# roymor1/OptimalStrategiesAgainstGenerativeAttacks

Measured on AMD Instinct MI355X. Metric: GIM episodes/sec (64x64x3, m=1 n=5 k=10), higher is better.
Workload: dtype f32

## Files before the change

### optimalstrategiesagainstgenerativeattacks_amd/csrc/conv_igemm.hip

```cpp
#include <stdlib.h>

#include "common.h"
#include <type_traits>

#define PM_MAX_PIXELS 16
#define PM_MIN_IMAGES 32
#define BK 16

struct Geo {
    int N, H, W, logH, logW;
    int Hin, Win;
    int ups;
    int s_in;
    int s_in_x;
    int off_y, off_x;
    int Th, Tw;
    int KF;
    int KFw;
    int wa_base, wa_step, wb_base, wb_step;
    int os, py, px;
    int pc, pc_kind, pc_K;
    int pm;
    unsigned long long pm_perm;
    unsigned long long pm_perm_cls[4];
// ... 1377 lines not shown

__global__ __launch_bounds__(256) void xfold_weights_kernel(const float* __restrict__ w, float* __restrict__ wx, int Cout, int Cin, int K, int J) {
    const int KW = K + J - 1;
    const long long total = (long long)J * Cin * K * KW * Cout;
    for (long long i = (long long)blockIdx.x * 256 + threadIdx.x; i < total; i += (long long)gridDim.x * 256) {
        const int co = (int)(i % Cout);
        long long r = i / Cout;
        const int u = (int)(r % KW); r /= KW;
        const int a = (int)(r % K); r /= K;
        const int ci = (int)(r % Cin), j = (int)(r / Cin);
        const int b = u - j;
        wx[i] = (b >= 0 && b < K) ? w[(((long long)co * K + (K - 1 - a)) * K + (K - 1 - b)) * Cin + ci] : 0.f;
    }
}

extern "C" int gim_conv2d_xfold_weights(const float* w, float* wx, int Cout, int Cin, int KH, int J, void* stream) {
    GIM_CHECK_ARG(w && wx && Cout > 0 && Cin > 0 && KH > 0 && (KH & 1) && J >= 2 && (J & (J - 1)) == 0, "xfold_weights: bad args");
    const long long total = (long long)J * Cin * KH * (KH + J - 1) * Cout;
    const int blocks = (int)((total + 255) / 256 < 2048 ? (total + 255) / 256 : 2048);
    hipLaunchKernelGGL(xfold_weights_kernel, dim3(blocks), dim3(256), 0, (hipStream_t)stream, w, wx, Cout, Cin, KH, J);
    return gim_check_launch("gim_conv2d_xfold_weights");
}

static int check_shape(const gim_conv_shape* s) {
    GIM_CHECK_ARG(s != nullptr, "conv: null shape");
    GIM_CHECK_ARG(s->N > 0 && s->Cin > 0 && s->Cout > 0, "conv: non-positive dims");
    GIM_CHECK_ARG(s->KH > 0 && (s->KH & 1), "conv: KH must be odd");
    GIM_CHECK_ARG(s->ups == 0 || s->ups == 1, "conv: ups must be 0 or 1");
    GIM_CHECK_ARG(ilog2_exact(s->H) >= 0 && ilog2_exact(s->W) >= 0, "conv: H and W must be powers of two");
    GIM_CHECK_ARG(!s->ups || (s->H >= 2 && s->W >= 2), "conv: ups needs H, W >= 2");
    GIM_CHECK_ARG(!s->pool || (!s->ups && s->H >= 2 && s->W >= 2 && s->wfold), "conv: pool needs ups == 0, H, W >= 2 and folded weights");
    GIM_CHECK_ARG(!s->wfold || s->pool || s->ups, "conv: wfold only with pool or ups");
    GIM_CHECK_ARG((long long)s->N * s->H * s->W < (1ll << 31), "conv: too many output pixels");
    GIM_CHECK_ARG(s->prec >= 0 && s->prec <= 2, "conv: prec must be 0 (fp32 MFMA), 1 (fp16 operands, fp32 accumulate; saturating) or 2 (the same, non-saturating)");
    return GIM_OK;
}

static void geo_grid(Geo& g, int N, int H, int W) {
    g.N = N; g.H = H; g.W = W; g.logH = ilog2_exact(H); g.logW = ilog2_exact(W);
}

static Geo geo_plain(const gim_conv_shape* s, bool flip) {
    Geo g{};
    const int pad = (s->KH - 1) / 2;
    geo_grid(g, s->N, s->H, s->W);
    g.ups = flip ? 0 : s->ups;
    g.Hin = s->H >> g.ups; g.Win = s->W >> g.ups;
    g.s_in = g.s_in_x = 1; g.off_y = g.off_x = -pad; g.Th = g.Tw = g.KF = g.KFw = s->KH;
    g.wa_base = g.wb_base = flip ? s->KH - 1 : 0;
    g.wa_step = g.wb_step = flip ? -1 : 1;
    g.os = 1;
    return g;
// ... 299 lines not shown
static int fwd_call(ConvCall& c, const float* x, const float* w, const float* bias, const float* sigma, const float* residual, float* y,
                    const gim_conv_shape* s) {
    c = ConvCall{};
    ConvP& p = c.p;
    const bool up_fold = s->ups && s->wfold;
    int rc = convp_begin(p, s->pool ? geo_s2(s, false) : (up_fold ? geo_pc(s, 0) : geo_plain(s, false)), s->Cin, s->Cout, s->Cin, 0, s,
                         "conv: one image of the gathered tensor exceeds 2 GiB (32-bit buffer offsets)");
    if (rc) return rc;
    p.x = x; p.w = w; p.bias = bias; p.sigma = sigma; p.res = residual; p.mask_x = nullptr; p.y = y;
    p.Cin_w = s->Cin;
    p.pre_slope = s->pre_slope; p.mask_slope = 1.f; p.out_scale = s->pool ? 0.25f : 1.f; p.res_ups = s->res_ups;
    GIM_CHECK_ARG(s->post_slope >= 0.f && s->post_slope <= 1.f, "conv fwd: post_slope must be in [0, 1] (0 or 1 = none)");
    p.post_slope = (s->post_slope > 0.f) ? s->post_slope : 1.f;
    p.f16 = s->prec;
    c.y_elems = (size_t)s->N * (s->H >> s->pool) * (s->W >> s->pool) * s->Cout;
    GIM_CHECK_ARG(c.y_elems * sizeof(float) <= 0x7FFFFFF0ull, "conv: one image of the output exceeds 2 GiB (32-bit buffer offsets)");
    c.bmode = 0;
    c.gen = ((s->Cin % BK) != 0 || ((uintptr_t)x & 15) || ((uintptr_t)w & 15)) ? 1 : 0;
    return GIM_OK;
}

extern "C" int gim_conv2d_fwd(const float* x, const float* w, const float* bias, const float* sigma, const float* residual,
                              float* y, const gim_conv_shape* s, void* stream) {
    int rc = check_shape(s);
    if (rc) return rc;
    GIM_CHECK_ARG(x && w && y, "conv fwd: null pointer");
    if (tiny_route(s)) {
        gim_tiny_fwd(x, w, bias, sigma, residual, y, s, (hipStream_t)stream);
        return gim_check_launch("gim_conv2d_fwd");
    }
    size_t xi, yi;
    image_elems(s, false, xi, yi);
    gim_conv_shape a, b;
    if (split_batch(*s, xi > yi ? xi : yi, a, b)) {
        const size_t ri = s->res_ups ? yi / 4 : yi;
        rc = gim_conv2d_fwd(x, w, bias, sigma, residual, y, &a, stream);
        if (rc) return rc;
        return gim_conv2d_fwd(x + a.N * xi, w, bias, sigma, residual ? residual + a.N * ri : nullptr, y + a.N * yi, &b, stream);
    }
    ConvCall c;
    rc = fwd_call(c, x, w, bias, sigma, residual, y, s);
    return rc ? rc : plan_and_run(c, stream, "gim_conv2d_fwd");
}

static Geo geo_strided(const gim_infer_conv* s) {
    Geo g{};
    const int pad = (s->KH - 1) / 2;
// ... 49 lines not shown
    if (rc) return rc;
    p.x = dy; p.w = w; p.bias = nullptr; p.sigma = sigma; p.res = res_half; p.res_scale = res_scale; p.mask_x = mask_x; p.y = dx;
    p.Cin_w = s->Cin;
    p.pre_slope = 1.f; p.mask_slope = s->pre_slope; p.out_scale = s->pool ? 0.25f : 1.f; p.res_ups = 0;
    p.post_slope = 1.f;
    c.y_elems = (size_t)s->N * (s->H >> (up_fold ? 1 : 0)) * (s->W >> (up_fold ? 1 : 0)) * s->Cin;
    GIM_CHECK_ARG(c.y_elems * sizeof(float) <= 0x7FFFFFF0ull, "conv: one image of the output exceeds 2 GiB (32-bit buffer offsets)");
    const bool gen = (s->Cout % BK) != 0 || ((uintptr_t)dy & 15);
    const bool bscalar = (s->Cin % 4) != 0 || ((uintptr_t)w & 15);
    p.f16 = transposed ? s->prec : 0;
    if (transposed) {
        GIM_CHECK_ARG(!gen && !((uintptr_t)w & 15), "conv dgrad (transposed weights): Cout % 16 == 0 and 16-byte aligned operands required");
        p.Cin_w = s->Cout;
        p.tune_kind = 4;
        c.bmode = 0; c.gen = 0;
    } else {
        c.bmode = 1; c.gen = (gen ? 1 : 0) | (bscalar ? 2 : 0);
    }
    return GIM_OK;
}

static int dgrad_impl(const float* dy, const float* w, const float* sigma, const float* mask_x, float* dx,
                      const gim_conv_shape* s, void* stream, bool transposed, const float* res_half = nullptr, float res_scale = 0.f) {
    int rc = check_shape(s);
    if (rc) return rc;
    GIM_CHECK_ARG(dy && w && dx, "conv dgrad: null pointer");
    if (!transposed && !res_half && tiny_route(s)) {
        gim_tiny_dgrad(dy, w, sigma, mask_x, dx, s, (hipStream_t)stream);
        return gim_check_launch("gim_conv2d_dgrad");
    }
    size_t xi, yi;
    image_elems(s, true, xi, yi);
    gim_conv_shape a, b;
    if (split_batch(*s, xi > yi ? xi : yi, a, b)) {
        rc = dgrad_impl(dy, w, sigma, mask_x, dx, &a, stream, transposed, res_half, res_scale);
        if (rc) return rc;
        return dgrad_impl(dy + a.N * yi, w, sigma, mask_x ? mask_x + a.N * xi : nullptr, dx + a.N * xi, &b, stream, transposed,
                          res_half ? res_half + a.N * (xi / 4) : nullptr, res_scale);
    }
    ConvCall c;
    rc = dgrad_call(c, dy, w, sigma, mask_x, dx, s, transposed, res_half, res_scale);
    return rc ? rc : plan_and_run(c, stream, transposed ? "gim_conv2d_dgrad_t" : "gim_conv2d_dgrad");
}

extern "C" int gim_conv2d_dgrad(const float* dy, const float* w, const float* sigma, const float* mask_x, float* dx,
                                const gim_conv_shape* s, void* stream) {
    return dgrad_impl(dy, w, sigma, mask_x, dx, s, stream, false);
// ... 230 lines not shown
            for (int m = m0 + lane; m < m1; m += 64) sb += nar[(long long)m * Cn + part];
        if (part < 8) red[0][part][lane] = sb;
        __syncthreads();
        if (threadIdx.x < Cn) {
            float v = 0.f;
            for (int q = 0; q < 64; ++q) v += red[0][threadIdx.x][q];
            atomicAdd(&bias_out[threadIdx.x], v);
        }
    }
}

enum WgFamily { WG_MFMA = 0, WG_MFMA_F16, WG_TINY, WG_ROW, WG_NARROW };
enum WgCombine { WG_SLABS = 0, WG_ONE_SLAB, WG_ACC };
struct WgPlan {
    int family;
    int rows, cols, M;
    int ns;
    int atomic;
    int bm, bn, bk, xcd;
    int slices, mper;
    int gx, gy, gz;
    int table_hit;
};

static WgPlan wgrad_plan(const gim_conv_shape* s0, bool rows_form, int combine, bool aligned) {
    WgPlan q{};
    gim_conv_shape v = *s0;
    if (rows_form) {
        v.tune_tile = s0->tune_tile ? s0->tune_tile : -1;
        v.prec = 0;
    }
    const gim_conv_shape* s = &v;
    const bool up_fold = s->ups && s->wfold;
    const int KF = s->wfold ? s->KH + 1 : s->KH;
    q.rows = up_fold ? s->Cin : s->Cout;
    q.cols = KF * KF * (up_fold ? s->Cout : s->Cin);
    const long long M = (long long)s->N * (s->H >> (s->wfold ? 1 : 0)) * (s->W >> (s->wfold ? 1 : 0));
    q.M = (int)M;
    int target = s->tune_wgrad > 0 ? s->tune_wgrad : 0;
    int tile = s->tune_tile > 0 ? s->tune_tile : 0;
    if (!target && !tile && s->tune_tile == 0) {
        const int pcw = (s->pool ? 1 : 0) + (up_fold ? 2 : 0);
        const TuneEntry* te = tune_lookup(2, (int)M, q.rows, q.cols, s->KH, pcw);
        if (te) { target = te->ks; tile = te->tile; q.table_hit = 1; }
    }
    bool row_resident = false;
// ... 12 lines not shown
    const long long tiles = (long long)((q.cols + q.bn - 1) / q.bn) * ((q.rows + q.bm - 1) / q.bm);
    long long minpix = 512;
    if (!target) {
        target = 1024;
        if (tiles * ((M + 511) / 512) < 256) minpix = 128;
    } else {
        minpix = 64;
    }
    long long S = (target + tiles - 1) / tiles;
    const long long maxS = (M + minpix - 1) / minpix;
    if (S > maxS) S = maxS;
    if (S > 1024) S = 1024;
    if (S < 1) S = 1;
    long long mp = (M + S - 1) / S;
    mp = (mp + q.bk - 1) / q.bk * q.bk;
    q.ns = (int)((M + mp - 1) / mp);
    if (rows_form) {
        q.cols = s->KH * ((s->KH * s->Cin + 15) & ~15);
        q.bn = (q.bm == 32 || q.cols > 64) ? 128 : 64;
    }
    q.atomic = combine == WG_ACC || (combine == WG_ONE_SLAB && q.ns > 1);
    const bool plain = !rows_form && !s->wfold && !s->ups && !s->pool;
    const bool untuned = s->tune_tile == 0 && s->tune_wgrad == 0;
    if (!rows_form && combine != WG_SLABS && untuned && gim_tiny_shape(s)) {
        const dim3 g = gim_tiny_grid(s);
        q.family = WG_TINY;
        q.table_hit = q.bm = q.bn = 0;
        q.gx = g.x; q.gy = g.y; q.gz = 1;
        q.slices = q.gx * q.gy;
    } else if (plain && row_resident && q.atomic && s->KH == 3 && s->Cin % 32 == 0 && s->Cout % 128 == 0 && s->H * s->W >= 16 && s->W >= 4 && aligned) {
        q.family = WG_ROW;
        q.bm = 128; q.bn = 96;
        q.gx = 3 * (s->Cin / 32); q.gy = s->Cout / 128;
        const int wgs = q.gx * q.gy;
        long long Sr = ((row_target > 0 ? row_target : 1024) + wgs - 1) / wgs;
        const long long maxSr = (M + 127) / 128;
        if (Sr > maxSr) Sr = maxSr;
        if (Sr < 1) Sr = 1;
        mp = (M + Sr - 1) / Sr;
        mp = (mp + 15) / 16 * 16;
        q.slices = q.gz = (int)((M + mp - 1) / mp);
    } else if (plain && s->KH == 1 && q.atomic && (s->Cin <= 8 || s->Cout <= 8) && (s->Cin >= 16 || s->Cout >= 16) && M % NARROW_U == 0 && untuned) {
        q.family = WG_NARROW;
        q.table_hit = q.bm = q.bn = 0;
        mp = NARROW_MPER;
        q.slices = q.gx = (int)((M + NARROW_MPER - 1) / NARROW_MPER);
        q.gy = ((s->Cin <= 8 ? s->Cout : s->Cin) + 63) / 64;
        q.gz = 1;
    } else {
        q.family = f16 ? WG_MFMA_F16 : WG_MFMA;
        q.slices = q.ns;
        q.xcd = (q.ns >= 64 || (q.ns >= 8 && q.ns % 8 == 0)) ? 1 : 0;
        q.gx = (q.cols + q.bn - 1) / q.bn; q.gy = (q.rows + q.bm - 1) / q.bm;
        q.gz = q.xcd ? (q.ns + 7) / 8 * 8 : q.ns;
    }
    q.mper = (int)mp;
    return q;
}

extern "C" int gim_conv2d_wgrad_slabs(const gim_conv_shape* s) {
    if (check_shape(s)) return GIM_E_BADARG;
    return wgrad_plan(s, false, WG_SLABS, true).ns;
}

static int wgrad_call(WgP& p, WgPlan& q, const float* dy, const float* x, float* slabs, float* bias_slabs, int n_slabs, const gim_conv_shape* s,
                      bool prezeroed, bool rows) {
    int rc = check_shape(s);
    if (rc) return rc;
    GIM_CHECK_ARG(dy && x && slabs, "conv wgrad: null pointer");
    q = wgrad_plan(s, rows, prezeroed ? WG_ACC : (n_slabs == 1 ? WG_ONE_SLAB : WG_SLABS), !((uintptr_t)dy & 15) && !((uintptr_t)x & 15));
    if (!prezeroed) GIM_CHECK_ARG(n_slabs == 1 || n_slabs == q.ns, "conv wgrad: n_slabs must be 1 (atomic combine) or gim_conv2d_wgrad_slabs(shape)");
    const bool up_fold = s->ups && s->wfold;
    GIM_CHECK_ARG(!(up_fold && bias_slabs), "conv wgrad: the sub-pixel form does not produce the bias gradient (use gim_colsum)");
    p = WgP{};
    p.zero = zero_page();
    p.pos_inf = __builtin_inff();
    if (rows) p.g = geo_rows(s);
    else if (s->pool || up_fold) p.g = geo_s2(s, false);
    else p.g = geo_plain(s, false);
    if (up_fold) {
        p.dy = x; p.x = dy; p.Cin = s->Cout; p.Cout = s->Cin; p.pre_slope = 1.f; p.a_slope = s->pre_slope; p.pix = s->Cout;
    } else {
        p.dy = dy; p.x = x; p.Cin = s->Cin; p.Cout = s->Cout; p.pre_slope = s->pre_slope; p.a_slope = 1.f; p.pix = s->Cin;
    }
    p.slabs = slabs; p.bias_slabs = bias_slabs;
    p.M = q.M; p.Kcols = q.cols; p.mper = q.mper; p.ns = q.slices; p.xcd = q.xcd; p.atomic = q.atomic;
    if (rows) { p.Cin = (s->KH * s->Cin + 15) & ~15; p.pix = s->Cin; p.pre_slope = 1.f; }
    const unsigned long long xb = (unsigned long long)p.g.N * p.g.Hin * p.g.Win * p.pix * 4ull;
    GIM_CHECK_ARG(xb <= 0x7FFFFFF0ull, "conv wgrad: gathered tensor larger than 2 GiB (32-bit buffer offsets): split the batch");
    p.x_bytes = (unsigned)xb;
    return GIM_OK;
}

// ... 32 lines not shown
        const bool va = (p.Cout % 4 == 0) && !((uintptr_t)p.dy & 15);
        const bool vb = (p.Cin % 4 == 0) && !((uintptr_t)p.x & 15);
        const int bk = (q.bk == 32 && va && vb) ? 32 : BK;
        const bool fastb = vb && p.g.ups == 0 && ((p.g.H * p.g.W) & (bk - 1)) == 0;
        const bool f16 = q.family == WG_MFMA_F16 && va && vb && bk == 32, sat = s->prec != 2;
        if (f16 && fastb) hipLaunchKernelGGL((sat ? conv_wgrad_f16_kernel<true, true> : conv_wgrad_f16_kernel<true, false>), g, dim3(256), 0, st, p);
        else if (f16) hipLaunchKernelGGL((sat ? conv_wgrad_f16_kernel<false, true> : conv_wgrad_f16_kernel<false, false>), g, dim3(256), 0, st, p);
        else if (va && fastb) launch_wgrad<4, 4, true>(p, q.bm, q.bn, bk, g, st);
        else if (va && vb) launch_wgrad<4, 4, false>(p, q.bm, q.bn, bk, g, st);
        else if (va) launch_wgrad<4, 1, false>(p, q.bm, q.bn, bk, g, st);
        else if (vb) launch_wgrad<1, 4, false>(p, q.bm, q.bn, bk, g, st);
        else launch_wgrad<1, 1, false>(p, q.bm, q.bn, bk, g, st);
    }
    }
    return gim_check_launch("gim_conv2d_wgrad");
}

extern "C" int gim_conv2d_wgrad(const float* dy, const float* x, float* slabs, float* bias_slabs, int n_slabs,
                                const gim_conv_shape* s, void* stream) {
    return wgrad_impl(dy, x, slabs, bias_slabs, n_slabs, s, stream, false);
}

extern "C" int gim_conv2d_wgrad_acc(const float* dy, const float* x, float* acc, float* bias_acc, const gim_conv_shape* s, void* stream) {
    int rc = check_shape(s);
    if (rc) return rc;
    size_t xi, yi;
    image_elems(s, false, xi, yi);
    gim_conv_shape a, b;
    if (split_batch(*s, xi > yi ? xi : yi, a, b)) {
        rc = gim_conv2d_wgrad_acc(dy, x, acc, bias_acc, &a, stream);
        if (rc) return rc;
        return gim_conv2d_wgrad_acc(dy + a.N * yi, x + a.N * xi, acc, bias_acc, &b, stream);
    }
    return wgrad_impl(dy, x, acc, bias_acc, 1, s, stream, true);
}

extern "C" int gim_conv2d_wgrad_rows_acc(const float* dy, const float* xp, float* acc, float* bias_acc, const gim_conv_shape* s, void* stream) {
    int rc = rows_shape_ok(s);
    if (rc) return rc;
    GIM_CHECK_ARG(s->Cout % 4 == 0 && dy && xp && !((uintptr_t)dy & 15) && !((uintptr_t)xp & 15), "conv wgrad (rows form): Cout % 4 == 0 and 16-byte aligned operands required");
    return wgrad_impl(dy, xp, acc, bias_acc, 1, s, stream, true, true);
}

static void plan_row(int32_t* out, int table_hit, int bm, int bn, int slices, int gx, int gy, int gz, int form) {
    const int32_t v[8] = {table_hit, bm, bn, slices, gx, gy, gz, form};
    for (int i = 0; i < 8; ++i) out[i] = v[i];
}
// ... 42 lines not shown
```

### optimalstrategiesagainstgenerativeattacks_amd/csrc/conv_tiny.hip

```cpp
#include "common.h"

struct TinyP {
    const float* in;
    const float* w;
    const float* bias;
    const float* sigma;
    const float* res;
    float* out;
    float* out2;
    int N, H, W;
    float pre_slope;
    float post_slope;
    int res_ups;
};

constexpr int TT = GIM_TINY_TILE;

template <int K, int CI, int CO, bool FLIP>
__global__ __launch_bounds__(256) void conv_tiny_kernel(const TinyP p) {
    constexpr int PAD = (K - 1) / 2, TW = TT + K - 1;
    constexpr int CG = FLIP ? CO : CI, CP = FLIP ? CI : CO;
    __shared__ float xs[TW * TW * CG];
    const int t = threadIdx.x;
    const int tiles_x = (p.W + TT - 1) / TT;
    const int oy0 = (blockIdx.x / tiles_x) * TT, ox0 = (blockIdx.x % tiles_x) * TT, n = blockIdx.y;
    const float* img = p.in + (long long)n * p.H * p.W * CG;
    for (int idx = t; idx < TW * TW * CG; idx += 256) {
        const int c = idx % CG, rc = idx / CG, col = rc % TW, row = rc / TW;
        const int iy = oy0 + row - PAD, ix = ox0 + col - PAD;
        float v = 0.f;
        if ((unsigned)iy < (unsigned)p.H && (unsigned)ix < (unsigned)p.W) v = img[((long long)iy * p.W + ix) * CG + c];
        if (!FLIP) v = fmaxf(v, v * p.pre_slope);
        xs[idx] = v;
    }
    __syncthreads();
    const int ty = t >> 4, tx = t & 15;
    float acc[CP];
#pragma unroll
    for (int c = 0; c < CP; ++c) acc[c] = 0.f;
    for (int ta = 0; ta < K; ++ta) {
#pragma unroll
        for (int tb = 0; tb < K; ++tb) {
// ... 9 lines not shown
            }
        }
    }
    const int oy = oy0 + ty, ox = ox0 + tx;
    if (oy >= p.H || ox >= p.W) return;
    const float scale = p.sigma ? 1.0f / p.sigma[0] : 1.0f;
    const long long o = (((long long)n * p.H + oy) * p.W + ox) * CP;
#pragma unroll
    for (int c = 0; c < CP; ++c) {
        float v = acc[c] * scale;
        if (FLIP) {
            if (p.res) v *= (p.res[o + c] > 0.f ? 1.0f : p.pre_slope);
        } else {
            if (p.bias) v += p.bias[c];
            if (p.res) v += p.res_ups ? p.res[(((long long)n * (p.H >> 1) + (oy >> 1)) * (p.W >> 1) + (ox >> 1)) * CP + c] : p.res[o + c];
            v = fmaxf(v, v * p.post_slope);
        }
        p.out[o + c] = v;
    }
}

template <int K, int CI, int CO>
__global__ __launch_bounds__(256) void conv_tiny_wgrad_kernel(const TinyP p) {
    constexpr int PAD = (K - 1) / 2, TW = TT + K - 1, NT = K * K * CI, G = 256 / NT;
    static_assert(G >= 1, "one thread per (tap, channel)");
    __shared__ float xs[TW * TW * CI];
    __shared__ float dys[TT * TT * CO];
    const int t = threadIdx.x;
    const int tiles_x = (p.W + TT - 1) / TT;
    const int oy0 = (blockIdx.x / tiles_x) * TT, ox0 = (blockIdx.x % tiles_x) * TT, n = blockIdx.y;
    const float* img = p.in + (long long)n * p.H * p.W * CI;
    const float* dyi = p.res + (long long)n * p.H * p.W * CO;
    for (int idx = t; idx < TW * TW * CI; idx += 256) {
        const int c = idx % CI, rc = idx / CI, col = rc % TW, row = rc / TW;
        const int iy = oy0 + row - PAD, ix = ox0 + col - PAD;
        float v = 0.f;
        if ((unsigned)iy < (unsigned)p.H && (unsigned)ix < (unsigned)p.W) v = img[((long long)iy * p.W + ix) * CI + c];
        xs[idx] = fmaxf(v, v * p.pre_slope);
    }
    for (int idx = t; idx < TT * TT * CO; idx += 256) {
        const int c = idx % CO, pp = idx / CO, oy = oy0 + (pp >> 4), ox = ox0 + (pp & 15);
        dys[idx] = (oy < p.H && ox < p.W) ? dyi[((long long)oy * p.W + ox) * CO + c] : 0.f;
    }
    __syncthreads();
    __shared__ float red[256 * CO];
    if (t < G * NT) {
        const int grp = t / NT, id = t - grp * NT;
        const int ci = id % CI, tap = id / CI, tb = tap % K, ta = tap / K;
        float acc[CO];
#pragma unroll
        for (int c = 0; c < CO; ++c) acc[c] = 0.f;
        for (int pp = grp; pp < TT * TT; pp += G) {
            const float xv = xs[(((pp >> 4) + ta) * TW + (pp & 15) + tb) * CI + ci];
#pragma unroll
            for (int c = 0; c < CO; ++c) acc[c] += dys[pp * CO + c] * xv;
        }
#pragma unroll
        for (int c = 0; c < CO; ++c) red[(grp * NT + id) * CO + c] = acc[c];
    }
    __syncthreads();
    for (int o = t; o < NT * CO; o += 256) {
        const int id = o / CO, c = o - id * CO;
        float v = 0.f;
        for (int gq = 0; gq < G; ++gq) v += red[(gq * NT + id) * CO + c];
        const int ci = id % CI, tap = id / CI, tb = tap % K, ta = tap / K;
        atomicAdd(&p.out[((c * K + ta) * K + tb) * CI + ci], v);
    }
    if (p.out2 && t >= 256 - CO) {
        const int c = t - (256 - CO);
        float s = 0.f;
        for (int pp = 0; pp < TT * TT; ++pp) s += dys[pp * CO + c];
        atomicAdd(&p.out2[c], s);
    }
}

bool gim_tiny_shape(const gim_conv_shape* s) {
    if (s->N > 65535) return false;
    return !s->ups && !s->pool && !s->wfold && s->Cin == s->Cout && (s->Cin == 3 || s->Cin == 1) && (s->KH == 3 || s->KH == 9);
}

dim3 gim_tiny_grid(const gim_conv_shape* s) { return dim3(((s->H + TT - 1) / TT) * ((s->W + TT - 1) / TT), s->N); }

template <bool FLIP>
static void tiny_launch(const TinyP& p, const gim_conv_shape* s, hipStream_t st) {
    const dim3 g = gim_tiny_grid(s);
    if (s->KH == 3 && s->Cin == 3) hipLaunchKernelGGL((conv_tiny_kernel<3, 3, 3, FLIP>), g, dim3(256), 0, st, p);
    else if (s->KH == 9 && s->Cin == 3) hipLaunchKernelGGL((conv_tiny_kernel<9, 3, 3, FLIP>), g, dim3(256), 0, st, p);
    else if (s->KH == 3) hipLaunchKernelGGL((conv_tiny_kernel<3, 1, 1, FLIP>), g, dim3(256), 0, st, p);
    else hipLaunchKernelGGL((conv_tiny_kernel<9, 1, 1, FLIP>), g, dim3(256), 0, st, p);
}

void gim_tiny_fwd(const float* x, const float* w, const float* bias, const float* sigma, const float* res, float* y,
                  const gim_conv_shape* s, hipStream_t st) {
    TinyP p{};
    p.in = x; p.w = w; p.bias = bias; p.sigma = sigma; p.res = res; p.out = y;
    p.N = s->N; p.H = s->H; p.W = s->W; p.pre_slope = s->pre_slope; p.post_slope = s->post_slope > 0.f ? s->post_slope : 1.f; p.res_ups = s->res_ups;
    tiny_launch<false>(p, s, st);
}

void gim_tiny_dgrad(const float* dy, const float* w, const float* sigma, const float* mask_x, float* dx, const gim_conv_shape* s,
                    hipStream_t st) {
    TinyP p{};
    p.in = dy; p.w = w; p.sigma = sigma; p.res = mask_x; p.out = dx;
    p.N = s->N; p.H = s->H; p.W = s->W; p.pre_slope = s->pre_slope; p.post_slope = 1.f;
    tiny_launch<true>(p, s, st);
}

void gim_tiny_wgrad_acc(const float* dy, const float* x, float* acc, float* bias_acc, const gim_conv_shape* s, hipStream_t st) {
    const dim3 g = gim_tiny_grid(s);
    TinyP p{};
    p.in = x; p.res = dy; p.out = acc; p.out2 = bias_acc;
    p.N = s->N; p.H = s->H; p.W = s->W; p.pre_slope = s->pre_slope;
    if (s->KH == 3 && s->Cin == 3) hipLaunchKernelGGL((conv_tiny_wgrad_kernel<3, 3, 3>), g, dim3(256), 0, st, p);
    else if (s->KH == 9 && s->Cin == 3) hipLaunchKernelGGL((conv_tiny_wgrad_kernel<9, 3, 3>), g, dim3(256), 0, st, p);
    else if (s->KH == 3) hipLaunchKernelGGL((conv_tiny_wgrad_kernel<3, 1, 1>), g, dim3(256), 0, st, p);
    else hipLaunchKernelGGL((conv_tiny_wgrad_kernel<9, 1, 1>), g, dim3(256), 0, st, p);
}
```

### optimalstrategiesagainstgenerativeattacks_amd/csrc/norm.hip

```cpp
#include "common.h"

template <int VEC, int CB>
struct NormCfg {
    static constexpr int CL = CB / VEC;
    static constexpr int HG = 256 / CL;
};

template <int VEC>
__device__ __forceinline__ void ld_vec(const float* p, float (&v)[VEC]) {
    if constexpr (VEC == 4) {
        const f32x4 t = *reinterpret_cast<const f32x4*>(p);
        v[0] = t[0]; v[1] = t[1]; v[2] = t[2]; v[3] = t[3];
    } else {
        v[0] = p[0];
    }
}
template <int VEC>
__device__ __forceinline__ void st_vec(float* p, const float (&v)[VEC]) {
    if constexpr (VEC == 4) {
        f32x4 t = {v[0], v[1], v[2], v[3]};
        *reinterpret_cast<f32x4*>(p) = t;
    } else {
        p[0] = v[0];
    }
// ... 137 lines not shown
    group_reduce<VEC, CB>(s2, red, cl, hg);
    if (!ok) return;
    if (hg == 0) {
#pragma unroll
        for (int e = 0; e < VEC; ++e) {
            dscale_nc[(long long)n * C + c + e] = s2[e];
            dshift_nc[(long long)n * C + c + e] = s1[e];
        }
    }
    const float inv_hw = 1.0f / (float)HW;
    for (int i = hg; i < HW; i += HG) {
        float g[VEC], v[VEC], o[VEC];
        ld_vec<VEC>(dy + off + (long long)i * C, g);
        ld_vec<VEC>(x + off + (long long)i * C, v);
#pragma unroll
        for (int e = 0; e < VEC; ++e) {
            const float xh = (v[e] - mean[e]) * invd[e];
            o[e] = sc[e] * ((g[e] - s1[e] * inv_hw) * invd[e] - xh * s2[e] * c2[e]);
        }
        st_vec<VEC>(dx + off + (long long)i * C, o);
    }
}

static int norm_fwd_impl(const float* x, const float* scale, const float* shift, const float* residual, float* y,
                         float* stats, int N, int HW, int C, int mode, float eps, float post_slope, void* stream) {
    GIM_CHECK_ARG(x && scale && shift && y && stats, "norm_fwd: null pointer");
    GIM_CHECK_ARG(N > 0 && HW > 0 && C > 0 && (mode == 0 || mode == 1), "norm_fwd: bad dims");
    const bool vec = (C % 4 == 0) && !(((uintptr_t)x | (uintptr_t)y | (uintptr_t)residual) & 15);
    hipStream_t st = (hipStream_t)stream;
    if (vec) hipLaunchKernelGGL((norm_fwd_kernel<4, 64>), dim3((C + 63) / 64, N), dim3(256), 0, st, x, scale, shift, residual, y, stats, HW, C, mode, eps, post_slope);
    else if (C <= 4) hipLaunchKernelGGL((norm_fwd_kernel<1, 4>), dim3(1, N), dim3(256), 0, st, x, scale, shift, residual, y, stats, HW, C, mode, eps, post_slope);
    else hipLaunchKernelGGL((norm_fwd_kernel<1, 64>), dim3((C + 63) / 64, N), dim3(256), 0, st, x, scale, shift, residual, y, stats, HW, C, mode, eps, post_slope);
    return gim_check_launch("gim_norm_fwd");
}

extern "C" int gim_norm_fwd(const float* x, const float* scale, const float* shift, const float* residual, float* y,
                            float* stats, int N, int HW, int C, int mode, float eps, void* stream) {
    return norm_fwd_impl(x, scale, shift, residual, y, stats, N, HW, C, mode, eps, 1.0f, stream);
}

extern "C" int gim_norm_fwd_act(const float* x, const float* scale, const float* shift, const float* residual, float* y,
                                float* stats, int N, int HW, int C, int mode, float eps, float post_slope, void* stream) {
    GIM_CHECK_ARG(post_slope > 0.f && post_slope <= 1.f, "norm_fwd_act: post_slope must be in (0, 1]");
    return norm_fwd_impl(x, scale, shift, residual, y, stats, N, HW, C, mode, eps, post_slope, stream);
}

extern "C" int gim_norm_bwd(const float* dy, const float* x, const float* scale, const float* stats, float* dx,
                            float* dscale_nc, float* dshift_nc, int N, int HW, int C, int mode, void* stream) {
    GIM_CHECK_ARG(dy && x && scale && stats && dx && dscale_nc && dshift_nc, "norm_bwd: null pointer");
    GIM_CHECK_ARG(N > 0 && HW > 0 && C > 0 && (mode == 0 || mode == 1), "norm_bwd: bad dims");
    const bool vec = (C % 4 == 0) && !(((uintptr_t)x | (uintptr_t)dy | (uintptr_t)dx) & 15);
    hipStream_t st = (hipStream_t)stream;
    if (vec) hipLaunchKernelGGL((norm_bwd_kernel<4, 64>), dim3((C + 63) / 64, N), dim3(256), 0, st, dy, x, scale, stats, dx, dscale_nc, dshift_nc, HW, C, mode);
    else if (C <= 4) hipLaunchKernelGGL((norm_bwd_kernel<1, 4>), dim3(1, N), dim3(256), 0, st, dy, x, scale, stats, dx, dscale_nc, dshift_nc, HW, C, mode);
    else hipLaunchKernelGGL((norm_bwd_kernel<1, 64>), dim3((C + 63) / 64, N), dim3(256), 0, st, dy, x, scale, stats, dx, dscale_nc, dshift_nc, HW, C, mode);
    return gim_check_launch("gim_norm_bwd");
}
```

Baseline: 433.9.

## Rework tiny 3-channel convs with register-blocked rows and whole-image norm kernels

```diff
diff --git a/optimalstrategiesagainstgenerativeattacks_amd/csrc/conv_igemm.hip b/optimalstrategiesagainstgenerativeattacks_amd/csrc/conv_igemm.hip
--- a/optimalstrategiesagainstgenerativeattacks_amd/csrc/conv_igemm.hip
+++ b/optimalstrategiesagainstgenerativeattacks_amd/csrc/conv_igemm.hip
@@ -1423,12 +1423,13 @@
     return gim_check_launch("gim_conv2d_xfold_weights");
 }
 
-static int check_shape(const gim_conv_shape* s) {
+static int check_shape(const gim_conv_shape* s, bool any_size = false) {
     GIM_CHECK_ARG(s != nullptr, "conv: null shape");
     GIM_CHECK_ARG(s->N > 0 && s->Cin > 0 && s->Cout > 0, "conv: non-positive dims");
     GIM_CHECK_ARG(s->KH > 0 && (s->KH & 1), "conv: KH must be odd");
     GIM_CHECK_ARG(s->ups == 0 || s->ups == 1, "conv: ups must be 0 or 1");
-    GIM_CHECK_ARG(ilog2_exact(s->H) >= 0 && ilog2_exact(s->W) >= 0, "conv: H and W must be powers of two");
+    GIM_CHECK_ARG((ilog2_exact(s->H) >= 0 && ilog2_exact(s->W) >= 0) || (any_size && s->H > 0 && s->W > 0 && (!s->res_ups || !((s->H | s->W) & 1))),
+                  "conv: H and W must be powers of two (the 3 -> 3 / 1 -> 1 direct image kernels: any size, even with a half-resolution residual)");
     GIM_CHECK_ARG(!s->ups || (s->H >= 2 && s->W >= 2), "conv: ups needs H, W >= 2");
     GIM_CHECK_ARG(!s->pool || (!s->ups && s->H >= 2 && s->W >= 2 && s->wfold), "conv: pool needs ups == 0, H, W >= 2 and folded weights");
     GIM_CHECK_ARG(!s->wfold || s->pool || s->ups, "conv: wfold only with pool or ups");
@@ -1774,7 +1775,7 @@
 
 extern "C" int gim_conv2d_fwd(const float* x, const float* w, const float* bias, const float* sigma, const float* residual,
                               float* y, const gim_conv_shape* s, void* stream) {
-    int rc = check_shape(s);
+    int rc = check_shape(s, s && tiny_route(s));
     if (rc) return rc;
     GIM_CHECK_ARG(x && w && y, "conv fwd: null pointer");
     if (tiny_route(s)) {
@@ -1870,7 +1871,7 @@
 
 static int dgrad_impl(const float* dy, const float* w, const float* sigma, const float* mask_x, float* dx,
                       const gim_conv_shape* s, void* stream, bool transposed, const float* res_half = nullptr, float res_scale = 0.f) {
-    int rc = check_shape(s);
+    int rc = check_shape(s, s && !transposed && !res_half && tiny_route(s));
     if (rc) return rc;
     GIM_CHECK_ARG(dy && w && dx, "conv dgrad: null pointer");
     if (!transposed && !res_half && tiny_route(s)) {
@@ -2147,6 +2148,10 @@
     int gx, gy, gz;
     int table_hit;
 };
+
+static bool tiny_wgrad_route(const gim_conv_shape* s, bool rows_form, int combine) {
+    return !rows_form && combine != WG_SLABS && s->tune_tile == 0 && s->tune_wgrad == 0 && gim_tiny_shape(s);
+}
 
 static WgPlan wgrad_plan(const gim_conv_shape* s0, bool rows_form, int combine, bool aligned) {
     WgPlan q{};
@@ -2205,7 +2210,7 @@
     q.atomic = combine == WG_ACC || (combine == WG_ONE_SLAB && q.ns > 1);
     const bool plain = !rows_form && !s->wfold && !s->ups && !s->pool;
     const bool untuned = s->tune_tile == 0 && s->tune_wgrad == 0;
-    if (!rows_form && combine != WG_SLABS && untuned && gim_tiny_shape(s)) {
+    if (tiny_wgrad_route(s, rows_form, combine)) {
         const dim3 g = gim_tiny_grid(s);
         q.family = WG_TINY;
         q.table_hit = q.bm = q.bn = 0;
@@ -2248,10 +2253,11 @@
 
 static int wgrad_call(WgP& p, WgPlan& q, const float* dy, const float* x, float* slabs, float* bias_slabs, int n_slabs, const gim_conv_shape* s,
                       bool prezeroed, bool rows) {
-    int rc = check_shape(s);
+    const int combine = prezeroed ? WG_ACC : (n_slabs == 1 ? WG_ONE_SLAB : WG_SLABS);
+    int rc = check_shape(s, s && tiny_wgrad_route(s, rows, combine));
     if (rc) return rc;
     GIM_CHECK_ARG(dy && x && slabs, "conv wgrad: null pointer");
-    q = wgrad_plan(s, rows, prezeroed ? WG_ACC : (n_slabs == 1 ? WG_ONE_SLAB : WG_SLABS), !((uintptr_t)dy & 15) && !((uintptr_t)x & 15));
+    q = wgrad_plan(s, rows, combine, !((uintptr_t)dy & 15) && !((uintptr_t)x & 15));
     if (!prezeroed) GIM_CHECK_ARG(n_slabs == 1 || n_slabs == q.ns, "conv wgrad: n_slabs must be 1 (atomic combine) or gim_conv2d_wgrad_slabs(shape)");
     const bool up_fold = s->ups && s->wfold;
     GIM_CHECK_ARG(!(up_fold && bias_slabs), "conv wgrad: the sub-pixel form does not produce the bias gradient (use gim_colsum)");
@@ -2330,7 +2336,7 @@
 }
 
 extern "C" int gim_conv2d_wgrad_acc(const float* dy, const float* x, float* acc, float* bias_acc, const gim_conv_shape* s, void* stream) {
-    int rc = check_shape(s);
+    int rc = check_shape(s, s && tiny_wgrad_route(s, false, WG_ACC));
     if (rc) return rc;
     size_t xi, yi;
     image_elems(s, false, xi, yi);
diff --git a/optimalstrategiesagainstgenerativeattacks_amd/csrc/conv_tiny.hip b/optimalstrategiesagainstgenerativeattacks_amd/csrc/conv_tiny.hip
--- a/optimalstrategiesagainstgenerativeattacks_amd/csrc/conv_tiny.hip
+++ b/optimalstrategiesagainstgenerativeattacks_amd/csrc/conv_tiny.hip
@@ -12,12 +12,130 @@
     float pre_slope;
     float post_slope;
     int res_ups;
+    int tiles_per_wg;
 };
 
 constexpr int TT = GIM_TINY_TILE;
+constexpr int QW = 4;
+constexpr int RS = 80;
+constexpr int TINY_WG_CAP = 160;
+
+template <int R>
+__device__ __forceinline__ void ld_row(const float* src, float (&xr)[4 * R]) {
+#pragma unroll
+    for (int r = 0; r < R; ++r) {
+        const f32x4 q = reinterpret_cast<const f32x4*>(src)[r];
+        xr[4 * r] = q[0]; xr[4 * r + 1] = q[1]; xr[4 * r + 2] = q[2]; xr[4 * r + 3] = q[3];
+    }
+}
+
+__device__ __forceinline__ void fma_sw(float& acc, float x, float w) { asm("v_fmac_f32_e32 %0, %1, %2" : "+v"(acc) : "s"(w), "v"(x)); }
+
+__device__ __forceinline__ void fma_vv(float& acc, float a, float b) { asm("v_fmac_f32_e32 %0, %1, %2" : "+v"(acc) : "v"(a), "v"(b)); }
+
+template <int K, int C, int NT, bool ACT>
+__device__ __forceinline__ void fill_tile(float* xs, const float* img, int oy0, int ox0, int H, int W, float slope, int t) {
+    constexpr int PAD = (K - 1) / 2, TW = TT + K - 1, NIT = (TW * TW * C + NT - 1) / NT;
+    float v[NIT];
+#pragma unroll
+    for (int i = 0; i < NIT; ++i) {
+        const int idx = t + i * NT, c = idx % C, rc = idx / C, col = rc % TW, row = rc / TW;
+        const int iy = oy0 + row - PAD, ix = ox0 + col - PAD;
+        v[i] = 0.f;
+        if (idx < TW * TW * C && (unsigned)iy < (unsigned)H && (unsigned)ix < (unsigned)W) v[i] = img[((long long)iy * W + ix) * C + c];
+    }
+#pragma unroll
+    for (int i = 0; i < NIT; ++i) {
+        const int idx = t + i * NT, c = idx % C, rc = idx / C, col = rc % TW, row = rc / TW;
+        if (idx < TW * TW * C) xs[row * RS + col * C + c] = ACT ? fmaxf(v[i], v[i] * slope) : v[i];
+    }
+}
 
 template <int K, int CI, int CO, bool FLIP>
-__global__ __launch_bounds__(256) void conv_tiny_kernel(const TinyP p) {
+__global__ __launch_bounds__(64) void conv_tiny_kernel(const TinyP p) {
+    constexpr int TW = TT + K - 1;
+    constexpr int CG = FLIP ? CO : CI, CP = FLIP ? CI : CO;
+    constexpr int R = ((QW + K - 1) * CG + 3) / 4;
+    static_assert(TW * CG <= RS && (TT - QW) * CG + 4 * R <= RS, "tile row stride");
+    __shared__ __attribute__((aligned(16))) float xs[TW * RS];
+    const int t = threadIdx.x;
+    const int tiles_x = (p.W + TT - 1) / TT;
+    const int oy0 = (blockIdx.x / tiles_x) * TT, ox0 = (blockIdx.x % tiles_x) * TT, n = blockIdx.y;
+    fill_tile<K, CG, 64, !FLIP>(xs, p.in + (long long)n * p.H * p.W * CG, oy0, ox0, p.H, p.W, p.pre_slope, t);
+    const int ty = t >> 2, tx = (t & 3) * QW;
+    const int oy = oy0 + ty, ox = ox0 + tx;
+    const long long o = (((long long)n * p.H + oy) * p.W + ox) * CP;
+    float ep[QW][CP];
+#pragma unroll
+    for (int px = 0; px < QW; ++px)
+#pragma unroll
+        for (int c = 0; c < CP; ++c) {
+            float v = FLIP ? 1.f : 0.f;
+            if (p.res && oy < p.H && ox + px < p.W) {
+                if (!FLIP && p.res_ups) v = p.res[(((long long)n * (p.H >> 1) + (oy >> 1)) * (p.W >> 1) + ((ox + px) >> 1)) * CP + c];
+                else v = p.res[o + px * CP + c];
+            }
+            ep[px][c] = v;
+        }
+    __syncthreads();
+    float acc[QW][CP];
+#pragma unroll
+    for (int px = 0; px < QW; ++px)
+#pragma unroll
+        for (int c = 0; c < CP; ++c) acc[px][c] = 0.f;
+    for (int ta = 0; ta < K; ++ta) {
+        float xr[4 * R];
+        ld_row<R>(&xs[(ty + ta) * RS + tx * CG], xr);
+        const float* wrow = p.w + (FLIP ? K - 1 - ta : ta) * K * CI;
+#pragma unroll
+        for (int tb = 0; tb < K; ++tb) {
+            const int wb = FLIP ? K - 1 - tb : tb;
+#pragma unroll
+            for (int cg = 0; cg < CG; ++cg)
+#pragma unroll
+                for (int cp = 0; cp < CP; ++cp) {
+                    const int co = FLIP ? cg : cp, ci = FLIP ? cp : cg;
+                    const float wv = wrow[(co * K * K + wb) * CI + ci];
+#pragma unroll
+                    for (int px = 0; px < QW; ++px) fma_sw(acc[px][cp], xr[(px + tb) * CG + cg], wv);
+                }
+        }
+    }
+    if (oy >= p.H) return;
+    const float scale = p.sigma ? 1.0f / p.sigma[0] : 1.0f;
+#pragma unroll
+    for (int px = 0; px < QW; ++px)
+#pragma unroll
+        for (int c = 0; c < CP; ++c) {
+            float v = acc[px][c] * scale;
+            if (FLIP) {
+                if (p.res) v *= (ep[px][c] > 0.f ? 1.0f : p.pre_slope);
+            } else {
+                if (p.bias) v += p.bias[c];
+                v += ep[px][c];
+                v = fmaxf(v, v * p.post_slope);
+            }
+            acc[px][c] = v;
+        }
+    if ((p.W & 3) == 0 && !((uintptr_t)p.out & 15)) {
+        if (ox >= p.W) return;
+#pragma unroll
+        for (int r = 0; r < CP; ++r) {
+            const f32x4 q = {acc[(4 * r) / CP][(4 * r) % CP], acc[(4 * r + 1) / CP][(4 * r + 1) % CP], acc[(4 * r + 2) / CP][(4 * r + 2) % CP],
+                             acc[(4 * r + 3) / CP][(4 * r + 3) % CP]};
+            reinterpret_cast<f32x4*>(p.out + o)[r] = q;
+        }
+    } else {
+#pragma unroll
+        for (int px = 0; px < QW; ++px)
+            if (ox + px < p.W)
+#pragma unroll
+                for (int c = 0; c < CP; ++c) p.out[o + px * CP + c] = acc[px][c];
+    }
+}
+
+template <int K, int CI, int CO, bool FLIP>
+__global__ __launch_bounds__(256) void conv_tiny_px_kernel(const TinyP p) {
     constexpr int PAD = (K - 1) / 2, TW = TT + K - 1;
     constexpr int CG = FLIP ? CO : CI, CP = FLIP ? CI : CO;
     __shared__ float xs[TW * TW * CG];
@@ -73,55 +191,87 @@
 
 template <int K, int CI, int CO>
 __global__ __launch_bounds__(256) void conv_tiny_wgrad_kernel(const TinyP p) {
-    constexpr int PAD = (K - 1) / 2, TW = TT + K - 1, NT = K * K * CI, G = 256 / NT;
-    static_assert(G >= 1, "one thread per (tap, channel)");
-    __shared__ float xs[TW * TW * CI];
-    __shared__ float dys[TT * TT * CO];
+    constexpr int TW = TT + K - 1, R = ((QW + K - 1) * CI + 3) / 4, RD = (QW * CO + 3) / 4;
+    constexpr int PG = 256 / K;
+    constexpr int NQ = TT * TT / QW;
+    constexpr int ACC = K * CI * CO;
+    constexpr int CH = ACC < 27 ? ACC : 27, ROUNDS = ACC / CH;
+    static_assert(TW * CI <= RS && (TT - QW) * CI + 4 * R <= RS && ACC % CH == 0 && K * CH <= 256, "wgrad tiling");
+    __shared__ __attribute__((aligned(16))) float xs[TW * RS];
+    __shared__ __attribute__((aligned(16))) float dys[TT * TT * CO];
+    __shared__ float red[256 * CH];
     const int t = threadIdx.x;
-    const int tiles_x = (p.W + TT - 1) / TT;
-    const int oy0 = (blockIdx.x / tiles_x) * TT, ox0 = (blockIdx.x % tiles_x) * TT, n = blockIdx.y;
-    const float* img = p.in + (long long)n * p.H * p.W * CI;
-    const float* dyi = p.res + (long long)n * p.H * p.W * CO;
-    for (int idx = t; idx < TW * TW * CI; idx += 256) {
-        const int c = idx % CI, rc = idx / CI, col = rc % TW, row = rc / TW;
-        const int iy = oy0 + row - PAD, ix = ox0 + col - PAD;
-        float v = 0.f;
-        if ((unsigned)iy < (unsigned)p.H && (unsigned)ix < (unsigned)p.W) v = img[((long long)iy * p.W + ix) * CI + c];
-        xs[idx] = fmaxf(v, v * p.pre_slope);
-    }
-    for (int idx = t; idx < TT * TT * CO; idx += 256) {
-        const int c = idx % CO, pp = idx / CO, oy = oy0 + (pp >> 4), ox = ox0 + (pp & 15);
-        dys[idx] = (oy < p.H && ox < p.W) ? dyi[((long long)oy * p.W + ox) * CO + c] : 0.f;
-    }
-    __syncthreads();
-    __shared__ float red[256 * CO];
-    if (t < G * NT) {
-        const int grp = t / NT, id = t - grp * NT;
-        const int ci = id % CI, tap = id / CI, tb = tap % K, ta = tap / K;
-        float acc[CO];
-#pragma unroll
-        for (int c = 0; c < CO; ++c) acc[c] = 0.f;
-        for (int pp = grp; pp < TT * TT; pp += G) {
-            const float xv = xs[(((pp >> 4) + ta) * TW + (pp & 15) + tb) * CI + ci];
-#pragma unroll
-            for (int c = 0; c < CO; ++c) acc[c] += dys[pp * CO + c] * xv;
-        }
-#pragma unroll
-        for (int c = 0; c < CO; ++c) red[(grp * NT + id) * CO + c] = acc[c];
-    }
-    __syncthreads();
-    for (int o = t; o < NT * CO; o += 256) {
-        const int id = o / CO, c = o - id * CO;
-        float v = 0.f;
-        for (int gq = 0; gq < G; ++gq) v += red[(gq * NT + id) * CO + c];
-        const int ci = id % CI, tap = id / CI, tb = tap % K, ta = tap / K;
-        atomicAdd(&p.out[((c * K + ta) * K + tb) * CI + ci], v);
-    }
-    if (p.out2 && t >= 256 - CO) {
-        const int c = t - (256 - CO);
-        float s = 0.f;
-        for (int pp = 0; pp < TT * TT; ++pp) s += dys[pp * CO + c];
-        atomicAdd(&p.out2[c], s);
+    const int ta = t % K, grp = t / K;
+    const int tiles_x = (p.W + TT - 1) / TT, tiles_img = tiles_x * ((p.H + TT - 1) / TT);
+    const long long tiles = (long long)tiles_img * p.N;
+    const long long l0 = (long long)blockIdx.x * p.tiles_per_wg;
+    const long long l1 = l0 + p.tiles_per_wg < tiles ? l0 + p.tiles_per_wg : tiles;
+    float acc[ACC], accb[CO];
+#pragma unroll
+    for (int i = 0; i < ACC; ++i) acc[i] = 0.f;
+#pragma unroll
+    for (int c = 0; c < CO; ++c) accb[c] = 0.f;
+    for (long long l = l0; l < l1; ++l) {
+        const int n = (int)(l / tiles_img), tile = (int)(l - (long long)n * tiles_img);
+        const int oy0 = (tile / tiles_x) * TT, ox0 = (tile % tiles_x) * TT;
+        const float* dyi = p.res + (long long)n * p.H * p.W * CO;
+        float dv[CO];
+#pragma unroll
+        for (int i = 0; i < CO; ++i) {
+            const int idx = t + i * 256, c = idx % CO, pp = idx / CO, oy = oy0 + (pp >> 4), ox = ox0 + (pp & 15);
+            dv[i] = (oy < p.H && ox < p.W) ? dyi[((long long)oy * p.W + ox) * CO + c] : 0.f;
+        }
+        __syncthreads();
+        fill_tile<K, CI, 256, true>(xs, p.in + (long long)n * p.H * p.W * CI, oy0, ox0, p.H, p.W, p.pre_slope, t);
+#pragma unroll
+        for (int i = 0; i < CO; ++i) dys[t + i * 256] = dv[i];
+        __syncthreads();
+        if (grp < PG)
+            for (int q = grp; q < NQ; q += PG) {
+                const int qy = q / (TT / QW), qx = (q % (TT / QW)) * QW;
+                float xr[4 * R], dq[4 * RD];
+                ld_row<R>(&xs[(qy + ta) * RS + qx * CI], xr);
+                ld_row<RD>(&dys[(qy * TT + qx) * CO], dq);
+#pragma unroll
+                for (int tb = 0; tb < K; ++tb)
+#pragma unroll
+                    for (int ci = 0; ci < CI; ++ci)
+#pragma unroll
+                        for (int co = 0; co < CO; ++co)
+#pragma unroll
+                            for (int px = 0; px < QW; ++px) fma_vv(acc[(tb * CI + ci) * CO + co], dq[px * CO + co], xr[(px + tb) * CI + ci]);
+#pragma unroll
+                for (int co = 0; co < CO; ++co)
+#pragma unroll
+                    for (int px = 0; px < QW; ++px) accb[co] += dq[px * CO + co];
+            }
+    }
+#pragma unroll
+    for (int r = 0; r < ROUNDS; ++r) {
+        __syncthreads();
+        if (grp < PG)
+#pragma unroll
+            for (int j = 0; j < CH; ++j) red[(grp * K + ta) * CH + j] = acc[r * CH + j];
+        __syncthreads();
+        if (t < K * CH) {
+            const int a = t / CH, j = t - a * CH;
+            float v = 0.f;
+            for (int g = 0; g < PG; ++g) v += red[(g * K + a) * CH + j];
+            const int e = r * CH + j, co = e % CO, ci = (e / CO) % CI, tb = e / (CO * CI);
+            atomicAdd(&p.out[((co * K + a) * K + tb) * CI + ci], v);
+        }
+    }
+    if (p.out2) {
+        __syncthreads();
+        if (grp < PG && ta == 0)
+#pragma unroll
+            for (int c = 0; c < CO; ++c) red[grp * CO + c] = accb[c];
+        __syncthreads();
+        if (t < CO) {
+            float v = 0.f;
+            for (int g = 0; g < PG; ++g) v += red[g * CO + t];
+            atomicAdd(&p.out2[t], v);
+        }
     }
 }
 
@@ -135,10 +285,10 @@
 template <bool FLIP>
 static void tiny_launch(const TinyP& p, const gim_conv_shape* s, hipStream_t st) {
     const dim3 g = gim_tiny_grid(s);
-    if (s->KH == 3 && s->Cin == 3) hipLaunchKernelGGL((conv_tiny_kernel<3, 3, 3, FLIP>), g, dim3(256), 0, st, p);
-    else if (s->KH == 9 && s->Cin == 3) hipLaunchKernelGGL((conv_tiny_kernel<9, 3, 3, FLIP>), g, dim3(256), 0, st, p);
-    else if (s->KH == 3) hipLaunchKernelGGL((conv_tiny_kernel<3, 1, 1, FLIP>), g, dim3(256), 0, st, p);
-    else hipLaunchKernelGGL((conv_tiny_kernel<9, 1, 1, FLIP>), g, dim3(256), 0, st, p);
+    if (s->KH == 9 && s->Cin == 3) hipLaunchKernelGGL((conv_tiny_kernel<9, 3, 3, FLIP>), g, dim3(64), 0, st, p);
+    else if (s->KH == 3 && s->Cin == 3) hipLaunchKernelGGL((conv_tiny_px_kernel<3, 3, 3, FLIP>), g, dim3(256), 0, st, p);
+    else if (s->KH == 3) hipLaunchKernelGGL((conv_tiny_px_kernel<3, 1, 1, FLIP>), g, dim3(256), 0, st, p);
+    else hipLaunchKernelGGL((conv_tiny_px_kernel<9, 1, 1, FLIP>), g, dim3(256), 0, st, p);
 }
 
 void gim_tiny_fwd(const float* x, const float* w, const float* bias, const float* sigma, const float* res, float* y,
@@ -158,10 +308,13 @@
 }
 
 void gim_tiny_wgrad_acc(const float* dy, const float* x, float* acc, float* bias_acc, const gim_conv_shape* s, hipStream_t st) {
-    const dim3 g = gim_tiny_grid(s);
+    const dim3 tg = gim_tiny_grid(s);
+    const long long tiles = (long long)tg.x * tg.y;
     TinyP p{};
     p.in = x; p.res = dy; p.out = acc; p.out2 = bias_acc;
     p.N = s->N; p.H = s->H; p.W = s->W; p.pre_slope = s->pre_slope;
+    p.tiles_per_wg = (int)((tiles + TINY_WG_CAP - 1) / TINY_WG_CAP);
+    const dim3 g((unsigned)((tiles + p.tiles_per_wg - 1) / p.tiles_per_wg));
     if (s->KH == 3 && s->Cin == 3) hipLaunchKernelGGL((conv_tiny_wgrad_kernel<3, 3, 3>), g, dim3(256), 0, st, p);
     else if (s->KH == 9 && s->Cin == 3) hipLaunchKernelGGL((conv_tiny_wgrad_kernel<9, 3, 3>), g, dim3(256), 0, st, p);
     else if (s->KH == 3) hipLaunchKernelGGL((conv_tiny_wgrad_kernel<3, 1, 1>), g, dim3(256), 0, st, p);
diff --git a/optimalstrategiesagainstgenerativeattacks_amd/csrc/norm.hip b/optimalstrategiesagainstgenerativeattacks_amd/csrc/norm.hip
--- a/optimalstrategiesagainstgenerativeattacks_amd/csrc/norm.hip
+++ b/optimalstrategiesagainstgenerativeattacks_amd/csrc/norm.hip
@@ -183,6 +183,148 @@
     }
 }
 
+constexpr int IMG_T = 1024, IMG_PX = 4;
+
+template <int NV>
+__device__ __forceinline__ void img_block_sum(float (&v)[NV], float* red) {
+    const int w = threadIdx.x >> 6;
+#pragma unroll
+    for (int e = 0; e < NV; ++e) v[e] = wave_sum(v[e]);
+    __syncthreads();
+    if ((threadIdx.x & 63) == 0)
+#pragma unroll
+        for (int e = 0; e < NV; ++e) red[w * NV + e] = v[e];
+    __syncthreads();
+#pragma unroll
+    for (int e = 0; e < NV; ++e) {
+        float a[16];
+#pragma unroll
+        for (int i = 0; i < 16; ++i) a[i] = red[i * NV + e];
+#pragma unroll
+        for (int h = 8; h > 0; h >>= 1)
+#pragma unroll
+            for (int i = 0; i < h; ++i) a[i] += a[i + h];
+        v[e] = a[0];
+    }
+}
+
+template <int C>
+__global__ __launch_bounds__(IMG_T) void norm_img_fwd_kernel(const float* __restrict__ x, const float* __restrict__ scale,
+                                                             const float* __restrict__ shift, const float* __restrict__ res,
+                                                             float* __restrict__ y, float* __restrict__ stats, int HW, int mode,
+                                                             float eps, float post_slope) {
+    __shared__ float red[16 * C];
+    const int n = blockIdx.x, t = threadIdx.x;
+    const long long base = (long long)n * HW * C;
+    float v[IMG_PX][C], mean[C], ssq[C];
+#pragma unroll
+    for (int j = 0; j < IMG_PX; ++j)
+#pragma unroll
+        for (int e = 0; e < C; ++e) v[j][e] = t + IMG_T * j < HW ? x[base + (long long)(t + IMG_T * j) * C + e] : 0.f;
+#pragma unroll
+    for (int e = 0; e < C; ++e) {
+        mean[e] = 0.f;
+#pragma unroll
+        for (int j = 0; j < IMG_PX; ++j) mean[e] += v[j][e];
+    }
+    img_block_sum<C>(mean, red);
+#pragma unroll
+    for (int e = 0; e < C; ++e) {
+        mean[e] /= (float)HW;
+        ssq[e] = 0.f;
+#pragma unroll
+        for (int j = 0; j < IMG_PX; ++j) {
+            const float d = t + IMG_T * j < HW ? v[j][e] - mean[e] : 0.f;
+            ssq[e] += d * d;
+        }
+    }
+    img_block_sum<C>(ssq, red);
+    float invd[C], sc[C], sh[C];
+#pragma unroll
+    for (int e = 0; e < C; ++e) {
+        float d, c2;
+        if (mode == 0) {
+            d = sqrtf(ssq[e] / (float)HW + eps);
+            c2 = 1.0f / ((float)HW * d);
+        } else {
+            const float sd = sqrtf(ssq[e] / (float)(HW - 1));
+            d = sd + eps;
+            c2 = sd > 0.f ? 1.0f / ((float)(HW - 1) * sd) : 0.f;
+        }
+        invd[e] = 1.0f / d;
+        const long long pi = (mode == 0) ? (long long)e : (long long)n * C + e;
+        sc[e] = scale[pi];
+        sh[e] = shift[pi];
+        if (t == 0) {
+            float* st = stats + ((long long)n * C + e) * 3;
+            st[0] = mean[e];
+            st[1] = invd[e];
+            st[2] = c2;
+        }
+    }
+#pragma unroll
+    for (int j = 0; j < IMG_PX; ++j)
+        if (t + IMG_T * j < HW)
+#pragma unroll
+            for (int e = 0; e < C; ++e) {
+                const long long i = base + (long long)(t + IMG_T * j) * C + e;
+                float o = sc[e] * ((v[j][e] - mean[e]) * invd[e]) + sh[e];
+                if (res) o += res[i];
+                y[i] = fmaxf(o, o * post_slope);
+            }
+}
+
+template <int C>
+__global__ __launch_bounds__(IMG_T) void norm_img_bwd_kernel(const float* __restrict__ dy, const float* __restrict__ x,
+                                                             const float* __restrict__ scale, const float* __restrict__ stats,
+                                                             float* __restrict__ dx, float* __restrict__ dscale_nc,
+                                                             float* __restrict__ dshift_nc, int HW, int mode) {
+    __shared__ float red[16 * 2 * C];
+    const int n = blockIdx.x, t = threadIdx.x;
+    const long long base = (long long)n * HW * C;
+    float g[IMG_PX][C], xh[IMG_PX][C], invd[C], c2[C], sc[C], s[2 * C];
+#pragma unroll
+    for (int j = 0; j < IMG_PX; ++j)
+#pragma unroll
+        for (int e = 0; e < C; ++e) {
+            const bool ok = t + IMG_T * j < HW;
+            const long long i = base + (long long)(t + IMG_T * j) * C + e;
+            g[j][e] = ok ? dy[i] : 0.f;
+            xh[j][e] = ok ? x[i] : 0.f;
+        }
+#pragma unroll
+    for (int e = 0; e < C; ++e) {
+        const float* st = stats + ((long long)n * C + e) * 3;
+        const float mean = st[0];
+        invd[e] = st[1];
+        c2[e] = st[2];
+        sc[e] = scale[(mode == 0) ? (long long)e : (long long)n * C + e];
+        s[e] = s[C + e] = 0.f;
+#pragma unroll
+        for (int j = 0; j < IMG_PX; ++j) {
+            xh[j][e] = (xh[j][e] - mean) * invd[e];
+            s[e] += g[j][e];
+            s[C + e] += g[j][e] * xh[j][e];
+        }
+    }
+    img_block_sum<2 * C>(s, red);
+    if (t == 0)
+#pragma unroll
+        for (int e = 0; e < C; ++e) {
+            dshift_nc[(long long)n * C + e] = s[e];
+            dscale_nc[(long long)n * C + e] = s[C + e];
+        }
+    const float inv_hw = 1.0f / (float)HW;
+#pragma unroll
+    for (int j = 0; j < IMG_PX; ++j)
+        if (t + IMG_T * j < HW)
+#pragma unroll
+            for (int e = 0; e < C; ++e)
+                dx[base + (long long)(t + IMG_T * j) * C + e] = sc[e] * ((g[j][e] - s[e] * inv_hw) * invd[e] - xh[j][e] * s[C + e] * c2[e]);
+}
+
+static bool norm_img_form(int HW, int C) { return C <= 3 && HW <= IMG_T * IMG_PX; }
+
 static int norm_fwd_impl(const float* x, const float* scale, const float* shift, const float* residual, float* y,
                          float* stats, int N, int HW, int C, int mode, float eps, float post_slope, void* stream) {
     GIM_CHECK_ARG(x && scale && shift && y && stats, "norm_fwd: null pointer");
@@ -190,6 +332,12 @@
     const bool vec = (C % 4 == 0) && !(((uintptr_t)x | (uintptr_t)y | (uintptr_t)residual) & 15);
     hipStream_t st = (hipStream_t)stream;
     if (vec) hipLaunchKernelGGL((norm_fwd_kernel<4, 64>), dim3((C + 63) / 64, N), dim3(256), 0, st, x, scale, shift, residual, y, stats, HW, C, mode, eps, post_slope);
+    else if (norm_img_form(HW, C)) {
+        const dim3 g(N), b(IMG_T);
+        if (C == 1) hipLaunchKernelGGL(norm_img_fwd_kernel<1>, g, b, 0, st, x, scale, shift, residual, y, stats, HW, mode, eps, post_slope);
+        else if (C == 2) hipLaunchKernelGGL(norm_img_fwd_kernel<2>, g, b, 0, st, x, scale, shift, residual, y, stats, HW, mode, eps, post_slope);
+        else hipLaunchKernelGGL(norm_img_fwd_kernel<3>, g, b, 0, st, x, scale, shift, residual, y, stats, HW, mode, eps, post_slope);
+    }
     else if (C <= 4) hipLaunchKernelGGL((norm_fwd_kernel<1, 4>), dim3(1, N), dim3(256), 0, st, x, scale, shift, residual, y, stats, HW, C, mode, eps, post_slope);
     else hipLaunchKernelGGL((norm_fwd_kernel<1, 64>), dim3((C + 63) / 64, N), dim3(256), 0, st, x, scale, shift, residual, y, stats, HW, C, mode, eps, post_slope);
     return gim_check_launch("gim_norm_fwd");
@@ -213,6 +361,12 @@
     const bool vec = (C % 4 == 0) && !(((uintptr_t)x | (uintptr_t)dy | (uintptr_t)dx) & 15);
     hipStream_t st = (hipStream_t)stream;
     if (vec) hipLaunchKernelGGL((norm_bwd_kernel<4, 64>), dim3((C + 63) / 64, N), dim3(256), 0, st, dy, x, scale, stats, dx, dscale_nc, dshift_nc, HW, C, mode);
+    else if (norm_img_form(HW, C)) {
+        const dim3 g(N), b(IMG_T);
+        if (C == 1) hipLaunchKernelGGL(norm_img_bwd_kernel<1>, g, b, 0, st, dy, x, scale, stats, dx, dscale_nc, dshift_nc, HW, mode);
+        else if (C == 2) hipLaunchKernelGGL(norm_img_bwd_kernel<2>, g, b, 0, st, dy, x, scale, stats, dx, dscale_nc, dshift_nc, HW, mode);
+        else hipLaunchKernelGGL(norm_img_bwd_kernel<3>, g, b, 0, st, dy, x, scale, stats, dx, dscale_nc, dshift_nc, HW, mode);
+    }
     else if (C <= 4) hipLaunchKernelGGL((norm_bwd_kernel<1, 4>), dim3(1, N), dim3(256), 0, st, dy, x, scale, stats, dx, dscale_nc, dshift_nc, HW, C, mode);
     else hipLaunchKernelGGL((norm_bwd_kernel<1, 64>), dim3((C + 63) / 64, N), dim3(256), 0, st, dy, x, scale, stats, dx, dscale_nc, dshift_nc, HW, C, mode);
     return gim_check_launch("gim_norm_bwd");
```

After: 437.3 (median of 6 runs). No clear change (+0.8%).
